# slinderman/pyglm

Measured on AMD Instinct MI355X. Metric: Gibbs sweeps/sec (full resample_model), higher is better.
Workload: dtype f64 (likelihood Gram: exact integer arithmetic on 13 i8 residue planes, CRT back to f64)

## Files before the change

### include/pyglm_hip.h

```cpp
#ifndef PYGLM_HIP_H
#define PYGLM_HIP_H
#include <stddef.h>
#include <stdint.h>
#ifdef __cplusplus
extern "C" {
#endif

#define PGL_ABI_VERSION 11

int pgl_abi_version(void);
const char* pgl_last_error(void);

int pgl_philox_words(uint64_t seed, uint32_t purpose, uint32_t j, uint64_t elem0, uint64_t stream, uint32_t* out, size_t n, void* hip_stream);

int pgl_pg_draw(const double* b, const double* z, double* out, size_t len, uint64_t seed, uint64_t stream, uint64_t elem0, void* hip_stream);

int pgl_design_matrix(const double* S, long lds, const double* basis, double* X, long ldx, double* Xt, long ldxt, int T, int N, int B, int R,
                      int clip, void* hip_stream);
int pgl_transpose(const double* src, long ld_src, double* dst, long ld_dst, int rows, int cols, void* hip_stream);

int pgl_activation(const double* Xt, long ldxt, const double* Wt, long ldw, double* Psi, long ldpsi, int T, int Dk, int nloc, void* hip_stream);

int pgl_pg_loglik(double* Psi, long ldpsi, const double* bias, const double* Y, long ldy, double* Omega, long ldo, double* Kappa, long ldk,
                  double* llpart, double* ll_out, int accumulate, int T, int nloc, int obs, double xi, uint64_t seed, uint64_t sweep,
                  uint64_t neuron0, uint64_t elem0, void* hip_stream);
int pgl_pg_loglik_partials(int T);
int pgl_pg_loglik_ex(double* Psi, long ldpsi, const double* bias, const double* Y, long ldy, double* Omega, long ldo, double* Kappa, long ldk,
                     double* llpart, double* ll_out, int accumulate, int T, int nloc, int obs, double xi, const double* param, const double* hooks,
                     long ldh, uint64_t seed, uint64_t sweep, uint64_t neuron0, uint64_t elem0, void* hip_stream);

int pgl_gaussian_stats(double* Psi, long ldpsi, const double* bias, const double* Y, long ldy, const double* inv_eta, double* Omega, long ldo,
                       double* Kappa, long ldk, double* part, double* sse_out, int accumulate, int T, int nloc, void* hip_stream);

int pgl_scaled_gram(const double* G0, long ldg, const double* inv_eta, double* J, long ldj, long strideJ, int D, int nz, void* hip_stream);

int pgl_weighted_gram(const double* X, long ldx, int x_cols, const double* W, long ldw, int Tp, int D, int nz, double* J, long ldj, long strideJ,
                      int accumulate, void* hip_stream);
int pgl_contract_tn(const double* A, long lda, int a_cols, const double* B, long ldb, int b_cols, double* C, long ldc, int M, int N, int K,
                    double alpha, double beta, void* hip_stream);
int pgl_contract_tn_batched(const double* A, long lda, long strideA, int a_cols, const double* B, long ldb, long strideB, int b_cols, double* C,
                            long ldc, long strideC, int M, int N, int K, int nbatch, const int* batch_k, double alpha, double beta, int tri,
                            int kernel, void* hip_stream);
int pgl_assemble_posterior(double* J, long ldj, long strideJ, const double* border_omega, const double* border_kappa, long ldb, const double* Jw,
                           const double* hw, const int* label, const double* Jb, const double* hb, int nb, int N, int B, void* hip_stream);

int pgl_i8_max_planes(void);
int pgl_i8_padded_rows(int D);
int pgl_i8_min_planes(int T);
int pgl_i8_norm_bits(int nplanes, int T);
double pgl_i8_norm_limit(int nplanes, int T);
size_t pgl_i8_plane_bytes(int D, int T);
size_t pgl_i8_residue_bytes(int D);
int pgl_i8_colstats(const double* X, long ldx, const double* Om, long ldo, int T, int D, int G, double* amax, double* sumsq, void* hip_stream);
int pgl_i8_scales(const double* amax, const double* sumsq, long ncols, int T, int nplanes, double* scale, void* hip_stream);
int pgl_i8_planes(const double* X, long ldx, const double* Om, long ldo, const double* scale, void* planes, int T, int D, int G, int nplanes,
                  long t0, void* hip_stream);
int pgl_i8_planes_t(const double* Xt, long ldt, const double* Om, long ldo, const double* scale, void* planes, int T, int D, int G, int nplanes,
                    long t0, void* hip_stream);
int pgl_i8_gram(const void* planes_x, const void* planes_wx, void* residues, int T, int D, int G, int nplanes, void* hip_stream);
int pgl_i8_gram_slice(const void* planes_x, int T_x, int t0, const void* planes_wx, void* residues, int T_slice, int T_total, int D, int G,
                      int nplanes, int accumulate, void* hip_stream);
int pgl_i8_crt(const void* residues, const double* scale_x, const double* scale_wx, double* J, long ldj, long strideJ, int T, int D, int G,
               int nplanes, int accumulate, void* hip_stream);

typedef struct {
    double* M; long ldj; long strideM;
    int nb, N, B;
    const int* perm;
    const double* u;
    const double* rho;
    const double* c0;
    int* a;
    const int* skip;
    int* d_idx; double* d_sign; int* d_cnt;
    int* batch_k;
    double* G;
    double* Lws;
    double* Ut; double* Wt; long ldu;
    int* status;
    int visit_order;
    double* logodds;
} pgl_flip_t;
int pgl_flip_kmax(void);
int pgl_flip_window_blocks(int B);
int pgl_flip_apply(const pgl_flip_t* s, void* hip_stream);
int pgl_flip_apply_chunk(const pgl_flip_t* s, int max_pivots, void* hip_stream);
int pgl_flip_apply_window(const pgl_flip_t* s, int window, void* hip_stream);
int pgl_flip_visit_order(const pgl_flip_t* s, const double* J, long ldj_src, long strideJ, void* hip_stream);
int pgl_flip_decide(const pgl_flip_t* s, int window, void* hip_stream);

typedef struct {
    const double* J; long ldj; long strideJ;
    const int* a;
    int* act; long ldact; int* na;
    double* Ac; long ldc; long strideC;
    double* hc;
    double* Tinv;
    const double* z; long ldz;
    double* W; double* b;
    int nb, N, B;
    int* status;
} pgl_chol_t;
int pgl_active_index(const pgl_chol_t* s, void* hip_stream);
int pgl_sample_weights(const pgl_chol_t* s, int na_max, void* hip_stream);

typedef struct {
    int T, Tp;
    const double* X;
    const double* Xt;
    const double* Y;
    double* Psi;
    double* OK;
    double* llpart;
    uint64_t elem0;
    int int8;
    int planes;
// ... 94 lines not shown
```

### pyglm_amd/_lib.py

```python
import ctypes
import os

_HERE = os.path.dirname(os.path.abspath(__file__))
LIB_PATH = os.path.join(_HERE, "lib", "libpyglm_hip.so")

c_p, c_l, c_i, c_d, c_u64, c_u32, c_sz = (ctypes.c_void_p, ctypes.c_long, ctypes.c_int, ctypes.c_double,
                                          ctypes.c_uint64, ctypes.c_uint32, ctypes.c_size_t)


class FlipState(ctypes.Structure):
    _fields_ = [("M", c_p), ("ldj", c_l), ("strideM", c_l), ("nb", c_i), ("N", c_i), ("B", c_i),
                ("perm", c_p), ("u", c_p), ("rho", c_p), ("c0", c_p), ("a", c_p), ("skip", c_p),
                ("d_idx", c_p), ("d_sign", c_p), ("d_cnt", c_p), ("batch_k", c_p), ("G", c_p), ("Lws", c_p),
                ("Ut", c_p), ("Wt", c_p), ("ldu", c_l), ("status", c_p), ("visit_order", c_i), ("logodds", c_p)]


class CholState(ctypes.Structure):
    _fields_ = [("J", c_p), ("ldj", c_l), ("strideJ", c_l), ("a", c_p), ("act", c_p), ("ldact", c_l), ("na", c_p),
                ("Ac", c_p), ("ldc", c_l), ("strideC", c_l), ("hc", c_p), ("Tinv", c_p), ("z", c_p), ("ldz", c_l),
                ("W", c_p), ("b", c_p), ("nb", c_i), ("N", c_i), ("B", c_i), ("status", c_p)]


class Dataset(ctypes.Structure):
    _fields_ = [("T", c_i), ("Tp", c_i), ("X", c_p), ("Xt", c_p), ("Y", c_p), ("Psi", c_p), ("OK", c_p), ("llpart", c_p), ("elem0", c_u64),
                ("int8", c_i), ("planes", c_i), ("sA", c_p), ("PA", c_p), ("omega_override", c_p), ("xmax", c_p),
                ("hooks", c_p)]


NSTAGES = 16


class StageTimes(ctypes.Structure):
    _fields_ = [("ms", c_d * NSTAGES), ("work", c_d * NSTAGES), ("calls", c_i * NSTAGES), ("pending", c_p), ("mask", c_u32)]


class Sweep(ctypes.Structure):
    _fields_ = [("N", c_i), ("B", c_i), ("n0", c_i), ("nloc", c_i), ("nb", c_i), ("obs", c_i), ("xi", c_d), ("visit_order", c_i),
                ("planes", c_i), ("i8_group", c_i), ("datasets", ctypes.POINTER(Dataset)), ("ndatasets", c_i),
                ("a", c_p), ("W", c_p), ("b", c_p), ("rho", c_p), ("Jw", c_p), ("hw", c_p), ("label", c_p), ("Jb", c_p), ("hb", c_p), ("c0", c_p),
                ("perm", c_p), ("u", c_p), ("z", c_p), ("inv_eta", c_p), ("G0", c_p), ("ll", c_p), ("status", c_p), ("logodds", c_p),
                ("Wt", c_p), ("bias", c_p), ("border", c_p), ("skip", c_p), ("c0_dense", c_p),
                ("Jbuf", c_p), ("Mtab", c_p), ("Ac", c_p), ("hc", c_p), ("Tinv", c_p), ("G", c_p), ("Lws", c_p), ("Ut", c_p), ("Wt_ws", c_p),
                ("d_idx", c_p), ("d_sign", c_p), ("d_cnt", c_p), ("batch_k", c_p), ("act", c_p), ("na", c_p),
                ("i8_PB", c_p), ("i8_R", c_p), ("i8_stat", c_p), ("i8_slice", c_i), ("i8_PAs", c_p), ("i8_Rx", c_p), ("i8_norm", c_p), ("nrun", c_i), ("nfirst", c_i),
                ("all_deterministic", c_i), ("init_rows_bound", c_i), ("active_rows_bound", c_i), ("flip_single_pass", c_i),
                ("times", ctypes.POINTER(StageTimes)), ("obs_param", c_p)]


SIGNATURES = {
    "pgl_abi_version": [],
    "pgl_last_error": [],
    "pgl_philox_words": [c_u64, c_u32, c_u32, c_u64, c_u64, c_p, c_sz, c_p],
    "pgl_pg_draw": [c_p, c_p, c_p, c_sz, c_u64, c_u64, c_u64, c_p],
    "pgl_design_matrix": [c_p, c_l, c_p, c_p, c_l, c_p, c_l, c_i, c_i, c_i, c_i, c_i, c_p],
    "pgl_transpose": [c_p, c_l, c_p, c_l, c_i, c_i, c_p],
    "pgl_activation": [c_p, c_l, c_p, c_l, c_p, c_l, c_i, c_i, c_i, c_p],
    "pgl_pg_loglik": [c_p, c_l, c_p, c_p, c_l, c_p, c_l, c_p, c_l, c_p, c_p, c_i, c_i, c_i, c_i, c_d, c_u64, c_u64, c_u64, c_u64, c_p],
    "pgl_pg_loglik_partials": [c_i],
    "pgl_pg_loglik_ex": [c_p, c_l, c_p, c_p, c_l, c_p, c_l, c_p, c_l, c_p, c_p, c_i, c_i, c_i, c_i, c_d, c_p, c_p, c_l, c_u64, c_u64, c_u64, c_u64, c_p],
    "pgl_gaussian_stats": [c_p, c_l, c_p, c_p, c_l, c_p, c_p, c_l, c_p, c_l, c_p, c_p, c_i, c_i, c_i, c_p],
    "pgl_scaled_gram": [c_p, c_l, c_p, c_p, c_l, c_l, c_i, c_i, c_p],
    "pgl_weighted_gram": [c_p, c_l, c_i, c_p, c_l, c_i, c_i, c_i, c_p, c_l, c_l, c_i, c_p],
    "pgl_i8_plane_bytes": [c_i, c_i],
    "pgl_i8_residue_bytes": [c_i],
    "pgl_i8_max_planes": [],
    "pgl_i8_padded_rows": [c_i],
    "pgl_i8_min_planes": [c_i],
    "pgl_i8_norm_bits": [c_i, c_i],
    "pgl_i8_norm_limit": [c_i, c_i],
    "pgl_i8_colstats": [c_p, c_l, c_p, c_l, c_i, c_i, c_i, c_p, c_p, c_p],
    "pgl_i8_scales": [c_p, c_p, c_l, c_i, c_i, c_p, c_p],
    "pgl_i8_planes": [c_p, c_l, c_p, c_l, c_p, c_p, c_i, c_i, c_i, c_i, c_l, c_p],
    "pgl_i8_planes_t": [c_p, c_l, c_p, c_l, c_p, c_p, c_i, c_i, c_i, c_i, c_l, c_p],
    "pgl_i8_gram": [c_p, c_p, c_p, c_i, c_i, c_i, c_i, c_p],
    "pgl_i8_gram_slice": [c_p, c_i, c_i, c_p, c_p, c_i, c_i, c_i, c_i, c_i, c_i, c_p],
    "pgl_i8_crt": [c_p, c_p, c_p, c_p, c_l, c_l, c_i, c_i, c_i, c_i, c_i, c_p],
    "pgl_contract_tn": [c_p, c_l, c_i, c_p, c_l, c_i, c_p, c_l, c_i, c_i, c_i, c_d, c_d, c_p],
    "pgl_contract_tn_batched": [c_p, c_l, c_l, c_i, c_p, c_l, c_l, c_i, c_p, c_l, c_l, c_i, c_i, c_i, c_i, c_p, c_d, c_d, c_i, c_i, c_p],
    "pgl_assemble_posterior": [c_p, c_l, c_l, c_p, c_p, c_l, c_p, c_p, c_p, c_p, c_p, c_i, c_i, c_i, c_p],
    "pgl_flip_kmax": [],
    "pgl_flip_window_blocks": [c_i],
    "pgl_flip_apply": [ctypes.POINTER(FlipState), c_p],
    "pgl_flip_apply_chunk": [ctypes.POINTER(FlipState), c_i, c_p],
    "pgl_flip_apply_window": [ctypes.POINTER(FlipState), c_i, c_p],
    "pgl_flip_visit_order": [ctypes.POINTER(FlipState), c_p, c_l, c_l, c_p],
    "pgl_flip_decide": [ctypes.POINTER(FlipState), c_i, c_p],
    "pgl_row_stats": [c_p, c_p, c_p, c_i, c_i, c_i, c_i, c_p],
    "pgl_sweep_dims": [c_i, c_i, c_i, ctypes.POINTER(c_i), ctypes.POINTER(c_i), ctypes.POINTER(c_i)],
    "pgl_sweep": [ctypes.POINTER(Sweep), c_u64, c_u64, c_p],
    "pgl_sweep_gram": [ctypes.POINTER(Sweep), c_i, c_i, c_p],
    "pgl_get_state": [ctypes.POINTER(Sweep), c_p, c_p, c_p, c_p, c_p, c_p],
    "pgl_stage_name": [c_i],
    "pgl_stage_times_collect": [ctypes.POINTER(StageTimes)],
    "pgl_active_index": [ctypes.POINTER(CholState), c_p],
    "pgl_sample_weights": [ctypes.POINTER(CholState), c_i, c_p],
    "pgl_ubench_mfma": [c_i, c_d, ctypes.POINTER(c_d), ctypes.POINTER(c_d), c_p],
    "pgl_generate_work_bytes": [c_i, c_i],
    "pgl_summary_fold": [c_p, c_l, c_p, c_p, c_p, c_p, c_i, c_i, c_i, c_i, c_d, c_p, c_p, c_l, c_p, c_p, c_p, c_p, c_i, c_p, c_d, c_p, c_p, c_p, c_p, c_i, c_p],
    "pgl_summary_state": [c_p, c_p, c_l, c_p, c_p, c_p, c_p, c_p, c_p, c_i, c_i, c_i, c_i, c_p],
    "pgl_summary_colsum": [c_p, c_l, c_i, c_i, c_p, c_p, c_i, c_p],
    "pgl_generate": [c_p, c_p, c_p, c_i, c_i, c_i, c_i, c_d, c_p, c_p, c_p, c_l, c_i, c_p, c_p, c_p],
    "pgl_simulate_work_bytes": [c_i, c_i, c_i],
    "pgl_simulate": [c_p, c_p, c_p, c_i, c_i, c_i, c_p, c_p, c_i, c_l, c_u64, c_p, c_p, c_l, c_p, c_p, c_l, c_i, c_p, c_p, c_p],
    "pgl_lagged_work_bytes": [c_i, c_i, c_i, c_i],
    "pgl_lagged_products": [c_p, c_l, c_l, c_i, c_i, c_i, c_i, c_i, c_p, c_l, c_i, c_i, c_p, c_p, c_p],
}

ABI_VERSION = 11
_lib = None


class PglError(RuntimeError):
    pass


def load():
    global _lib
    if _lib is not None:
        return _lib
    if not os.path.exists(LIB_PATH):
        raise PglError("libpyglm_hip.so not found at %s -- build it with `python -c 'import __graft_entry__ as g; g.build()'` "
                       "or `make -C pyglm_amd/csrc` (there is no CPU fallback)" % LIB_PATH)
    import torch
    lib = ctypes.CDLL(LIB_PATH)
    for name, args in SIGNATURES.items():
        fn = getattr(lib, name)
        fn.argtypes = args
        fn.restype = (ctypes.c_char_p if name in ("pgl_last_error", "pgl_stage_name") else ctypes.c_size_t if name in ("pgl_i8_plane_bytes", "pgl_i8_residue_bytes", "pgl_generate_work_bytes", "pgl_simulate_work_bytes", "pgl_lagged_work_bytes")
                      else ctypes.c_double if name == "pgl_i8_norm_limit" else ctypes.c_int)
# ... 30 lines not shown
```

### pyglm_amd/csrc/pgl_api.hip

```cpp
#include "pgl_common.h"
#include "pgl_obs.h"
#include <cstdarg>
#include <cstdio>

static thread_local char g_err[512] = "";
void pgl_set_error(const char* fmt, ...) {
    va_list ap;
    va_start(ap, fmt);
    vsnprintf(g_err, sizeof(g_err), fmt, ap);
    va_end(ap);
}

int pgl_device() {
    int dev = 0;
    if (hipGetDevice(&dev) != hipSuccess || dev < 0) dev = 0;
    return dev;
}
int pgl_device_cus(int dev) {
    static std::atomic<int> cus[PGL_MAX_DEVICES];
    const int slot = dev & (PGL_MAX_DEVICES - 1);
    int n = cus[slot].load(std::memory_order_relaxed);
    if (n <= 0) {
        if (hipDeviceGetAttribute(&n, hipDeviceAttributeMultiprocessorCount, dev) != hipSuccess || n <= 0) n = 256;
        cus[slot].store(n, std::memory_order_relaxed);
// ... 153 lines not shown
    return pgl_k_assemble_post(J, ldj, strideJ, border_omega, border_kappa, ldb, Jw, hw, label, Jb, hb, nb, N, B, ST(st));
}

size_t pgl_i8_plane_bytes(int D, int T) { return pgl_k_i8_plane_bytes(D, T); }
size_t pgl_i8_residue_bytes(int D) { return pgl_k_i8_residue_bytes(D); }
int pgl_i8_max_planes(void) { return pgl_k_i8_max_planes(); }
int pgl_i8_padded_rows(int D) { return pgl_k_i8_padded_rows(D); }
int pgl_i8_min_planes(int T) { return pgl_k_i8_min_planes(T); }
int pgl_i8_norm_bits(int nplanes, int T) { return pgl_k_i8_nu(nplanes, T); }
double pgl_i8_norm_limit(int nplanes, int T) { return pgl_k_i8_norm_limit(nplanes, T); }
#define PGL_CHECK_PLANES(np, T) PGL_CHECK_ARG((np) >= 1 && (np) <= pgl_k_i8_max_planes() && pgl_k_i8_nu((np), (T)) >= 8)
int pgl_i8_colstats(const double* X, long ldx, const double* Om, long ldo, int T, int D, int G, double* amax, double* sumsq, void* st) {
    PGL_CHECK_ARG(X && amax && sumsq && T > 0 && D > 0 && G >= 1 && G <= 8 && ldx >= D && (Om == nullptr ? G == 1 : ldo >= G));
    return pgl_k_i8_colstats(X, ldx, Om, ldo, T, D, G, amax, sumsq, ST(st));
}
int pgl_i8_scales(const double* amax, const double* sumsq, long ncols, int T, int nplanes, double* scale, void* st) {
    PGL_CHECK_ARG(amax && sumsq && scale && ncols > 0 && T > 0);
    PGL_CHECK_PLANES(nplanes, T);
    return pgl_k_i8_scales(amax, sumsq, ncols, T, nplanes, scale, ST(st));
}
int pgl_i8_planes(const double* X, long ldx, const double* Om, long ldo, const double* scale, void* planes, int T, int D, int G, int nplanes,
                  long t0, void* st) {
    PGL_CHECK_ARG(X && scale && planes && T > 0 && D > 0 && G > 0 && ldx >= D && (Om == nullptr || ldo >= G) && t0 >= 0);
    PGL_CHECK_ARG(Om != nullptr || G == 1);
    PGL_CHECK_PLANES(nplanes, T);
    return pgl_k_i8_planes(X, ldx, 0, Om, ldo, scale, static_cast<int8_t*>(planes), T, D, G, nplanes, t0, ST(st));
}
int pgl_i8_planes_t(const double* Xt, long ldt, const double* Om, long ldo, const double* scale, void* planes, int T, int D, int G, int nplanes,
                    long t0, void* st) {
    PGL_CHECK_ARG(Xt && scale && planes && T > 0 && D > 0 && G > 0 && ldt >= T && (Om == nullptr || ldo >= G) && t0 >= 0);
    PGL_CHECK_ARG(Om != nullptr || G == 1);
    PGL_CHECK_PLANES(nplanes, T);
    return pgl_k_i8_planes(Xt, ldt, 1, Om, ldo, scale, static_cast<int8_t*>(planes), T, D, G, nplanes, t0, ST(st));
}
int pgl_i8_gram(const void* planes_x, const void* planes_wx, void* residues, int T, int D, int G, int nplanes, void* st) {
    PGL_CHECK_ARG(planes_x && planes_wx && residues && T > 0 && D > 0 && G > 0);
    PGL_CHECK_PLANES(nplanes, T);
    return pgl_k_i8_gram(static_cast<const int8_t*>(planes_x), 0, 0, static_cast<const int8_t*>(planes_wx), static_cast<int8_t*>(residues), nullptr, T, D, G,
                         nplanes, 0, ST(st));
}
int pgl_i8_gram_slice(const void* planes_x, int T_x, int t0, const void* planes_wx, void* residues, int T_slice, int T_total, int D, int G, int nplanes,
                      int accumulate, void* st) {
    PGL_CHECK_ARG(planes_x && planes_wx && residues && T_slice > 0 && D > 0 && G > 0 && t0 >= 0 && t0 % 64 == 0 && T_total >= T_slice);
    PGL_CHECK_ARG(T_x == 0 || t0 + T_slice <= T_x);
    PGL_CHECK_PLANES(nplanes, T_total);
    return pgl_k_i8_gram(static_cast<const int8_t*>(planes_x), T_x > 0 ? pgl_k_i8_kp(T_x) : 0, T_x > 0 ? t0 / 64 : 0, static_cast<const int8_t*>(planes_wx),
                         static_cast<int8_t*>(residues), nullptr, T_slice, D, G, nplanes, accumulate, ST(st));
}
int pgl_i8_crt(const void* residues, const double* scale_x, const double* scale_wx, double* J, long ldj, long strideJ, int T, int D, int G,
               int nplanes, int accumulate, void* st) {
    PGL_CHECK_ARG(residues && scale_x && scale_wx && J && T > 0 && D > 0 && G > 0 && ldj >= D);
    PGL_CHECK_PLANES(nplanes, T);
    return pgl_k_i8_crt(static_cast<const int8_t*>(residues), nullptr, scale_x, scale_wx, J, ldj, strideJ, D, G, nplanes, accumulate, ST(st));
}

int pgl_summary_fold(const double* Psi, long ldn, const double* bias, const double* Y, double* llpart, double* ll_out, int accumulate, int T,
                     int nloc, int obs, double xi, const double* param, const double* hooks, long ldh, const double* inv_eta, double* rate_mean,
                     double* rate_M2, const int* link, int link0, const double* link_par, double link_par0, double* l_mean, double* l_M2,
                     double* lse_m, double* lse_s, int k, void* st) {
    PGL_CHECK_ARG(Psi && Y && llpart && ll_out && T > 0 && nloc > 0 && ldn >= nloc && obs >= 0 && obs <= 4 && k >= 1);
    PGL_CHECK_ARG(obs != 2 || inv_eta != nullptr);
    PGL_CHECK_ARG(obs == 2 || param != nullptr || obs == 0 || obs == 4 || (obs == 1 ? xi > 0 : xi >= 0));
    PGL_CHECK_ARG(obs != 4 || (hooks != nullptr && ldh >= nloc));
    PGL_CHECK_ARG((rate_mean == nullptr) == (rate_M2 == nullptr) && (link != nullptr || (link0 >= 0 && link0 <= 3)));
    PGL_CHECK_ARG((l_mean != nullptr) == (l_M2 != nullptr) && (l_mean != nullptr) == (lse_m != nullptr) && (l_mean != nullptr) == (lse_s != nullptr));
    PglSummaryFold f{};
    f.Psi = const_cast<double*>(Psi); f.ldpsi = ldn; f.bias = bias; f.Y = Y; f.ldy = ldn; f.llpart = llpart; f.T = T; f.nloc = nloc;
    f.obs = obs; f.xi = xi; f.param = param; f.hooks = obs == 4 ? hooks : nullptr; f.ldh = ldh; f.inv_eta = inv_eta;
    f.ll_out = ll_out; f.accumulate = accumulate;
    f.rmean = rate_mean; f.rM2 = rate_M2; f.link = link; f.link0 = link0; f.link_par = link_par; f.link_par0 = link_par0;
    f.lmean = l_mean; f.lM2 = l_M2; f.lse_m = lse_m; f.lse_s = lse_s; f.k = k;
    return pgl_k_summary_fold(f, ST(st));
}
int pgl_summary_state(const int* a, const double* Wt, long ldw, const double* bias, double* edge, double* w_mean, double* w_M2, double* b_mean,
                      double* b_M2, int N, int B, int nloc, int k, void* st) {
    PGL_CHECK_ARG(a && Wt && bias && edge && w_mean && w_M2 && b_mean && b_M2 && N > 0 && B > 0 && nloc > 0 && ldw >= nloc && k >= 1);
    return pgl_k_summary_state(a, Wt, ldw, bias, edge, w_mean, w_M2, b_mean, b_M2, N, B, nloc, k, ST(st));
}
int pgl_summary_colsum(const double* V, long ldv, int T, int nloc, double* part, double* out, int accumulate, void* st) {
    PGL_CHECK_ARG(V && part && out && T > 0 && nloc > 0 && ldv >= nloc);
    return pgl_k_summary_colsum(V, ldv, T, nloc, part, out, accumulate, ST(st));
}

int pgl_flip_kmax(void) { return pgl_k_flip_kmax(); }
int pgl_flip_window_blocks(int B) { return pgl_k_flip_window_blocks(B); }
int pgl_flip_apply(const pgl_flip_t* s, void* st) {
    PGL_CHECK_ARG(s && s->M && s->d_idx && s->d_sign && s->d_cnt && s->batch_k && s->G && s->Ut && s->Wt && s->status);
    PGL_CHECK_ARG(s->ldu >= (long)s->N * s->B + 2 && s->ldu % 2 == 0 && s->ldj >= (long)s->N * s->B + 2 && s->nb > 0);
    return pgl_k_flip_apply(*s, 0, 128, -1, ST(st));
}
int pgl_flip_apply_chunk(const pgl_flip_t* s, int max_pivots, void* st) {
    PGL_CHECK_ARG(s && s->M && s->d_idx && s->d_sign && s->d_cnt && s->batch_k && s->G && s->Lws && s->Ut && s->Wt && s->status);
    PGL_CHECK_ARG(s->ldu >= (long)s->N * s->B + 2 && s->ldu % 2 == 0 && s->ldj >= (long)s->N * s->B + 2 && s->nb > 0 && max_pivots > 0);
    return pgl_k_flip_apply(*s, 0, max_pivots, -1, ST(st));
}
int pgl_flip_visit_order(const pgl_flip_t* s, const double* J, long ldj_src, long strideJ, void* st) {
    PGL_CHECK_ARG(s && s->M && s->perm && J && s->visit_order && s->nb > 0 && ldj_src >= (long)s->N * s->B + 2 && s->ldj >= (long)s->N * s->B + 2);
    PGL_CHECK_ARG(s->B >= 1 && s->B <= 32);
    return pgl_k_flip_permute(*s, J, ldj_src, strideJ, ST(st));
}
int pgl_flip_apply_window(const pgl_flip_t* s, int window, void* st) {
    PGL_CHECK_ARG(s && s->M && s->d_idx && s->d_sign && s->d_cnt && s->batch_k && s->G && s->Ut && s->Wt && s->status);
    PGL_CHECK_ARG(s->ldu >= (long)s->N * s->B + 2 && s->ldu % 2 == 0 && s->ldj >= (long)s->N * s->B + 2 && s->nb > 0);
    PGL_CHECK_ARG(window >= 0);
    return pgl_k_flip_apply(*s, 1, 0, window, ST(st));
}
// ... 18 lines not shown
```

### pyglm_amd/csrc/pgl_common.h

```cpp
#pragma once
#include <hip/hip_runtime.h>
#include <stdint.h>
#include <stddef.h>
#include <atomic>
#include "../../include/pyglm_hip.h"

#define PGL_OK 0
#define PGL_ERR_ARG 1
#define PGL_ERR_HIP 2

void pgl_set_error(const char* fmt, ...);

#ifdef PGL_AB
#include <cstdlib>
inline int pgl_ab_int(const char* name, int dflt) { const char* e = getenv(name); return e ? atoi(e) : dflt; }
#else
constexpr int pgl_ab_int(const char*, int dflt) { return dflt; }
#endif

constexpr int PGL_MAX_DEVICES = 32;
int pgl_device();
int pgl_device_cus(int dev);
struct PglPerDevice {
    std::atomic<uint32_t> mask{0};
// ... 30 lines not shown
    double* C; long ldc; long strideC;
    const double* W; long ldw;
    int M, N, K;
    int a_cols, b_cols;
    int nbatch;
    int nz_total;
    double alpha, beta;
    int tri;
    const int* batch_k;
    int* sched;
    const int* batch_dim; int dim_off;
    int dim_mode;
    const int* batch_row_off;
    int pipe;
    int ksplit; long ks_rows; double* Cpart; long part_stride_z, part_stride_s;
};
enum PglGemmKind { PGL_GEMM_GRAM2 = 0, PGL_GEMM_PLAIN = 1, PGL_GEMM_TRI1 = 2, PGL_GEMM_SQUARES = 3 };
int pgl_launch_gemm(PglGemmKind kind, const PglGemmArgs& a, hipStream_t st);
int pgl_gram_split(const double* X, long ldx, int x_cols, const double* W, long ldw, int Tp, int D, int nz, double* J, long ldj, long strideJ, int accumulate,
                   long ks_rows, double* part, long part_stride_z, hipStream_t st);
bool pgl_update_supported(const PglGemmArgs& a);
int pgl_launch_update(const PglGemmArgs& a, hipStream_t st);
int pgl_launch_update_rows(const PglGemmArgs& a, int row0, int nrows, hipStream_t st);
int* pgl_sched_slot(hipStream_t st);

int pgl_k_philox_words(uint64_t, uint32_t, uint32_t, uint64_t, uint64_t, uint32_t*, size_t, hipStream_t);
int pgl_k_pg_draw(const double*, const double*, double*, size_t, uint64_t, uint64_t, uint64_t, hipStream_t);
int pgl_k_row_stats(const int* a, const double* W, double* out, int N, int B, int nloc, int n0, hipStream_t st);
int pgl_k_colsum_partials(const double* part, int nblk, int ncol, double* out, int accumulate, hipStream_t st);
int pgl_k_summary_state(const int* a, const double* Wt, long ldw, const double* bias, double* edge, double* wmean, double* wM2, double* bmean,
                        double* bM2, int N, int B, int nloc, int k, hipStream_t st);
int pgl_k_summary_colsum(const double* V, long ldv, int T, int nloc, double* part, double* out, int accumulate, hipStream_t st);
int pgl_k_scaled_gram(const double*, long, const double*, double*, long, long, int, int, hipStream_t);
int pgl_k_basis_conv(const double*, long, const double*, double*, long, double*, long, int, int, int, int, int, hipStream_t);
int pgl_k_transpose(const double*, long, double*, long, int, int, hipStream_t);
int pgl_k_assemble_post(double*, long, long, const double*, const double*, long, const double*, const double*, const int*, const double*,
                        const double*, int, int, int, hipStream_t);
size_t pgl_k_i8_plane_bytes(int, int);
size_t pgl_k_i8_residue_bytes(int);
int pgl_k_i8_max_planes(void);
int pgl_k_i8_padded_rows(int);
int pgl_k_i8_min_planes(int);
int pgl_k_i8_nu(int, int);
double pgl_k_i8_norm_limit(int, int);
int pgl_k_i8_colstats(const double*, long, const double*, long, int, int, int, double*, double*, hipStream_t);
int pgl_k_i8_scales(const double*, const double*, long, int, int, double*, hipStream_t);
int pgl_k_i8_colmax(const double*, long, int, int, double*, hipStream_t);
int pgl_k_i8_scales_bound(const double*, long, const double*, const double*, int, int, int, int, double*, hipStream_t);
int pgl_k_i8_colstats_scales(const double*, long, const double*, long, int, int, int, int, double*, double*, hipStream_t);
int pgl_k_i8_planes(const double*, long, int transposed, const double*, long, const double*, int8_t*, int, int, int, int, long t_base, hipStream_t);
int pgl_k_i8_gram(const int8_t*, long, int, const int8_t*, int8_t*, int8_t*, int, int, int, int, int, hipStream_t);
long pgl_k_i8_kp(int);
int pgl_k_i8_crt(const int8_t*, const int8_t*, const double*, const double*, double*, long, long, int, int, int, int, hipStream_t);
int pgl_k_flip_apply(const pgl_flip_t&, int, int, int, hipStream_t);
int pgl_k_flip_apply_pair(const pgl_flip_t&, int phase, int window, int* ws, hipStream_t);
int pgl_k_flip_permute(const pgl_flip_t&, const double*, long, long, hipStream_t);
int pgl_k_flip_decide(const pgl_flip_t&, int, hipStream_t);
int pgl_k_flip_pivot_list(const pgl_flip_t&, int*, long, int*, hipStream_t);
int pgl_k_flip_pivot_chunk(const pgl_flip_t&, const int*, long, const int*, int, int, hipStream_t);
int pgl_k_flip_kmax(void);
int pgl_k_flip_window_blocks(int);
int pgl_k_chol_index(const pgl_chol_t&, hipStream_t);
bool pgl_k_small_fits(int N, int B);
int pgl_k_small_max_rows(void);
int pgl_k_small_tail(const double* J, long ldj, long strideJ, int nb, int N, int B, const int* perm, const double* u, const double* rho, const double* c0,
                     int* a, const int* skip, const double* z, long ldz, double* W, double* b, int* status, double* logodds, hipStream_t st);
int pgl_k_chol_sample(const pgl_chol_t&, int, hipStream_t);
```

### pyglm_amd/csrc/pgl_i8gram.hip

```cpp
#include "pgl_common.h"
#include <cmath>
#include <type_traits>

namespace {

constexpr int NP = 15;
struct ModTable {
    int p[NP] = {256, 255, 253, 251, 247, 241, 239, 233, 229, 227, 223, 217, 211, 199, 197};
    int w[NP][NP] = {};
    int pinv[NP] = {};
    constexpr ModTable() {
        for (int q = 1; q < NP; ++q) {
            int prod = 1;
            for (int k = 0; k < q; ++k) {
                w[k][q] = prod > p[q] / 2 ? prod - p[q] : prod;
                prod = (prod * (p[k] % p[q])) % p[q];
            }
            int x = 1;
            while ((prod * x) % p[q] != 1) ++x;
            pinv[q] = x;
        }
    }
};
constexpr ModTable MT{};
__constant__ int c_mod[NP] = {256, 255, 253, 251, 247, 241, 239, 233, 229, 227, 223, 217, 211, 199, 197};

typedef int v4i __attribute__((ext_vector_type(4)));
typedef int v16i __attribute__((ext_vector_type(16)));
typedef __attribute__((address_space(3))) void* lds_ptr_t;
typedef const __attribute__((address_space(1))) void* glb_ptr_t;

constexpr int ELEM_BITS = 50;

constexpr int CS_COLS = 16, CS_LANES = 64, CS_G = 8, CS_ROWS = 4;
template <int G, bool WEIGHTED>
__global__ __launch_bounds__(CS_COLS * CS_LANES) void i8_colstats_kernel(const double* __restrict__ X, long ldx, const double* __restrict__ Om,
                                                                        long ldo, int T, int D, double* __restrict__ amax,
                                                                        double* __restrict__ ss) {
    constexpr int CH = CS_LANES * CS_ROWS;
    __shared__ double red[2][CS_LANES][CS_COLS + 1];
    __shared__ double oms[WEIGHTED ? CH : 1][WEIGHTED ? G : 1];
    const int tid = threadIdx.x, cl = tid % CS_COLS, tl = tid / CS_COLS, c = blockIdx.x * CS_COLS + cl;
    const bool live = c < D;
    const int tchunk = ((T + (int)gridDim.y - 1) / (int)gridDim.y + CH - 1) / CH * CH;
    const int tbeg = (int)blockIdx.y * tchunk;
    T = T < tbeg + tchunk ? T : tbeg + tchunk;
    amax += (long)blockIdx.y * G * D;
    ss += (long)blockIdx.y * G * D;
    double m[G], q[G];
#pragma unroll
    for (int g = 0; g < G; ++g) { m[g] = 0.0; q[g] = 0.0; }
    for (int t0 = tbeg; t0 < T; t0 += CH) {
        if (WEIGHTED) {
            __syncthreads();
            for (int e = tid; e < CH * G; e += CS_COLS * CS_LANES) {
                const int t = t0 + e / G;
                oms[e / G][e % G] = t < T ? Om[(long)t * ldo + e % G] : 0.0;
            }
            __syncthreads();
        }
        double x[CS_ROWS];
#pragma unroll
        for (int r = 0; r < CS_ROWS; ++r) {
            const int t = t0 + tl + r * CS_LANES;
            x[r] = (live && t < T) ? X[(long)t * ldx + c] : 0.0;
        }
#pragma unroll
        for (int r = 0; r < CS_ROWS; ++r)
#pragma unroll
            for (int g = 0; g < G; ++g) {
                const double v = WEIGHTED ? x[r] * oms[tl + r * CS_LANES][g] : x[r];
                m[g] = fmax(m[g], fabs(v));
                q[g] = fma(v, v, q[g]);
// ... 467 lines not shown
    asm volatile("s_getreg_b32 %0, hwreg(HW_REG_XCC_ID)" : "=s"(xcc));
    xcc &= 7u;
    for (;;) {
        __syncthreads();
        if (threadIdx.x == 0) {
            int w = -1, y = 0;
            for (int hop = 0; hop < 8 && w < 0; ++hop) {
                y = (int)((xcc + hop) & 7u);
                const int it = atomicAdd(&g.sched[y], 1);
                if (npx) { if (it < per_xcd) w = it; }
                else {
                    const long cand = ((long)(it / CH) * 8 + y) * CH + it % CH;
                    if (cand < total) w = (int)cand;
                }
            }
            if (w >= 0) {
                int tm, tn, gz, q, kpart = -1, tile;
                if (!npx) { const int pair = w / ntiles; tile = w % ntiles; gz = pair / g.np; q = pair % g.np; }
                else if (pieces) {
                    const int per_piece = npx * ntiles, per_plane = PGL_KPARTS(g) * per_piece, r = w % per_plane, r2 = r % per_piece;
                    q = w / per_plane; kpart = r / per_piece; gz = y + 8 * (r2 / ntiles); tile = r2 % ntiles;
                }
                else if (w < nfull) {
                    const int per_plane = npx * ntiles, r = w % per_plane;
                    q = w / per_plane; gz = y + 8 * (r / ntiles); tile = r % ntiles;
                } else {
                    const int r0 = w - nfull, j = r0 / (4 * ntiles), r = r0 % (4 * ntiles), grp = r / 128, within = r - grp * 128;
                    const int tg = min(32, ntiles - grp * 32);
                    kpart = within / tg;
                    tile = grp * 32 + within % tg;
                    gz = y + 8 * j; q = g.np - 1;
                }
                clustered_tile(tile, ntm, g.sbr, g.sbc, tm, tn);
                ticket[1] = gz; ticket[2] = tm; ticket[3] = tn; ticket[4] = kpart; ticket[5] = q;
            }
            ticket[0] = w;
        }
        __syncthreads();
        if (ticket[0] < 0) break;
        const int gz = __builtin_amdgcn_readfirstlane(ticket[1]), q = __builtin_amdgcn_readfirstlane(ticket[5]);
        const int tm = __builtin_amdgcn_readfirstlane(ticket[2]), tn = __builtin_amdgcn_readfirstlane(ticket[3]);
        const int kpart = __builtin_amdgcn_readfirstlane(ticket[4]);
        __syncthreads();
        i8_gram_item_big(g, gz, q, tm, tn, lds, kpart);
    }
}

struct CrtArgs {
    const int8_t* R;
    const double* sA; const double* sB;
    double* J; long ldj; long strideJ;
    int D, Dq, G, accumulate, np;
    const int8_t* Rx;
};

__device__ __forceinline__ double recip_scale(double x) {
    const long long b = __double_as_longlong(x);
    const bool pow2 = (b & 0x000FFFFFFFFFFFFFll) == 0 && b > 0x0010000000000000ll && b < 0x7FD0000000000000ll;
    return pow2 ? __longlong_as_double(0x7FE0000000000000ll - b) : 1.0 / x;
}

__global__ __launch_bounds__(256) void i8_crt_kernel(CrtArgs a) {
    const int j0 = (blockIdx.x * 256 + threadIdx.x) * 4, i = blockIdx.y, gz = blockIdx.z;
    if (j0 > i || i >= a.D) return;
    const int8_t* R = a.R + ((long)gz * a.np) * a.Dq * a.Dq + (long)i * a.Dq + j0;
    int w[NP];
#pragma unroll
    for (int q = 0; q < NP; ++q) w[q] = q < a.np ? *reinterpret_cast<const int*>(R + (long)q * a.Dq * a.Dq) : 0;
    int wx[3] = {0, 0, 0};
    if (a.Rx) {
        const int8_t* Rx = a.Rx + (long)gz * 3 * a.Dq * a.Dq + (long)i * a.Dq + j0;
#pragma unroll
        for (int k = 0; k < 3; ++k) wx[k] = *reinterpret_cast<const int*>(Rx + (long)k * a.Dq * a.Dq);
    }
    const double ra = recip_scale(a.sA[i]);
    double out[4];
#pragma unroll
    for (int e = 0; e < 4; ++e) {
        int v[NP];
#pragma unroll
        for (int q = 0; q < NP; ++q) v[q] = (int)(int8_t)((unsigned)w[q] >> (8 * e));
        if (a.Rx) {
            const int x = (int)(int8_t)((unsigned)wx[0] >> (8 * e)) + (int)(int8_t)((unsigned)wx[1] >> (8 * e)) + (int)(int8_t)((unsigned)wx[2] >> (8 * e));
#pragma unroll
            for (int q = 1; q < NP; ++q) if (q == a.np - 1) v[q] += x;
        }
#pragma unroll
        for (int q = 1; q < NP; ++q) {
            if (q < a.np) {
                const int p = MT.p[q];
                int u = v[q];
#pragma unroll
                for (int k = 0; k < q; ++k) u -= v[k] * MT.w[k][q];
                int t = u * MT.pinv[q] % p;
                if (t > p / 2) t -= p; else if (t < -(p / 2)) t += p;
                v[q] = t;
            }
        }
        double s = 0.0;
#pragma unroll
        for (int q = NP - 1; q >= 0; --q)
            if (q < a.np) s = s * (double)MT.p[q] + (double)v[q];
        const int j = j0 + e;
        const double rb = j < a.D ? recip_scale(a.sB[(long)gz * a.D + j]) : 0.0;
        out[e] = (s * ra) * rb;
    }
    double* dst = a.J + (long)gz * a.strideJ + (long)i * a.ldj + j0;
    if (j0 + 3 <= i && !a.accumulate && (reinterpret_cast<uintptr_t>(dst) % 16 == 0)) {
        *reinterpret_cast<d2_t*>(dst) = d2_t{out[0], out[1]};
        *reinterpret_cast<d2_t*>(dst + 2) = d2_t{out[2], out[3]};
    } else {
#pragma unroll
        for (int e = 0; e < 4; ++e)
            if (j0 + e <= i) dst[e] = a.accumulate ? dst[e] + out[e] : out[e];
    }
}

}

int pgl_k_i8_padded_rows(int D) { return (D + BT - 1) / BT * BT; }

static long pgl_i8_kp(int T) { const long k = ((long)T + 63) / 64 * 64; return k < 256 ? 256 : k; }

double pgl_k_i8_norm_limit(int nplanes, int T) {
    double l2 = 0.0;
    for (int q = 0; q < nplanes && q < NP; ++q) l2 += std::log2((double)MT.p[q]);
    const double lim = (std::exp2((l2 - 1.0) * 0.5) - std::sqrt((double)(T < 1 ? 1 : T)) - 1.0) / (1.0 + 1e-9);
    return lim > 0.0 ? lim : 0.0;
}
int pgl_k_i8_nu(int nplanes, int T) {
    const double lim = pgl_k_i8_norm_limit(nplanes, T);
    if (!(lim >= 2.0)) return 0;
    return (int)std::floor(std::log2(lim) - 1e-12);
}
int pgl_k_i8_max_planes(void) { return NP; }
int pgl_k_i8_min_planes(int T) {
    for (int k = 1; k <= NP; ++k)
        if (pgl_k_i8_nu(k, T) >= 50) return k;
    return NP + 1;
}

long pgl_k_i8_kp(int T) { return pgl_i8_kp(T); }
static int pgl_k_i8_kparts() { static const int v = pgl_ab_int("PGL_I8_KPARTS", 0); return v >= 2 && v <= 16 ? v : 0; }
static bool pgl_k_i8_split(int G, int nplanes) { return G % 8 == 0 && nplanes >= 2 && pgl_k_i8_kparts() == 0; }
size_t pgl_k_i8_plane_bytes(int D, int T) {
    const long Dq = pgl_k_i8_padded_rows(D), Kp = pgl_i8_kp(T);
    return (size_t)NP * Dq * Kp;
}
size_t pgl_k_i8_residue_bytes(int D) {
    const long Dq = pgl_k_i8_padded_rows(D);
    return (size_t)NP * Dq * Dq;
}

int pgl_k_i8_colstats(const double* X, long ldx, const double* Om, long ldo, int T, int D, int G, double* amax, double* ss, hipStream_t st) {
    if (G > CS_G || G < 1) { pgl_set_error("i8 colstats: %d weight columns per call (max %d)", G, CS_G); return PGL_ERR_ARG; }
    const dim3 grid((D + CS_COLS - 1) / CS_COLS), block(CS_COLS * CS_LANES);
#define PGL_CS(g_) case g_: hipLaunchKernelGGL((i8_colstats_kernel<g_, true>), grid, block, 0, st, X, ldx, Om, ldo, T, D, amax, ss); break;
    if (!Om) hipLaunchKernelGGL((i8_colstats_kernel<1, false>), grid, block, 0, st, X, ldx, Om, ldo, T, D, amax, ss);
    else switch (G) { PGL_CS(1) PGL_CS(2) PGL_CS(3) PGL_CS(4) PGL_CS(5) PGL_CS(6) PGL_CS(7) PGL_CS(8) default: break; }
#undef PGL_CS
    PGL_CHECK_LAUNCH();
    return PGL_OK;
}

constexpr int CS_NCH = 4;
int pgl_k_i8_colstats_scales(const double* X, long ldx, const double* Om, long ldo, int T, int D, int G, int nplanes, double* scratch, double* scale,
                             hipStream_t st) {
    if (G > CS_G || G < 1 || !Om) { pgl_set_error("i8 colstats+scales: %d weight columns per call (max %d)", G, CS_G); return PGL_ERR_ARG; }
// ... 34 lines not shown
    if (pgl_k_i8_nu(nplanes, T) < 8) { pgl_set_error("i8 scales: %d moduli leave no room for T = %d", nplanes, T); return PGL_ERR_ARG; }
    hipLaunchKernelGGL(i8_scales_kernel, dim3((unsigned)((n + 255) / 256)), dim3(256), 0, st, amax, ss, n, pgl_k_i8_norm_limit(nplanes, T), scale, 1);
    PGL_CHECK_LAUNCH();
    return PGL_OK;
}

int pgl_k_i8_planes(const double* X, long ldx, int transposed, const double* Om, long ldo, const double* scale, int8_t* P, int T, int D, int G,
                    int nplanes, long t_base, hipStream_t st) {
    const int Dq = pgl_k_i8_padded_rows(D);
    const long Kp = pgl_i8_kp(T);
    const bool aligned = (ldx % 2 == 0) && (reinterpret_cast<uintptr_t>(X) % 16 == 0);
    for (int g0 = 0; g0 < G; g0 += CS_G) {
        const int gz = G - g0 < CS_G ? G - g0 : CS_G;
        PlaneArgs a{X, ldx, transposed, Om ? Om + g0 : nullptr, ldo, scale + (long)g0 * D, P + (long)g0 * nplanes * Dq * Kp, T, D, Dq, Kp, nplanes, (unsigned)t_base};
        if (transposed && aligned)
            hipLaunchKernelGGL(i8_planes_t_kernel<256>, dim3((unsigned)((Kp + 255) / 256), Dq / PT_D), dim3(256), 0, st, a, gz);
        else
            hipLaunchKernelGGL(i8_planes_kernel<512>, dim3((unsigned)((Kp + 511) / 512), Dq / PT_D), dim3(512), 0, st, a, gz);
        PGL_CHECK_LAUNCH();
    }
    return PGL_OK;
}

int pgl_k_i8_gram(const int8_t* PA, long KpA, int ka0, const int8_t* PB, int8_t* R, int8_t* Rx, int T, int D, int G, int nplanes, int accumulate, hipStream_t st) {
    const int Dq = pgl_k_i8_padded_rows(D);
    const long Kp = pgl_i8_kp(T);
    if (KpA <= 0) { KpA = Kp; ka0 = 0; }
    const int nkt = (T + BKB - 1) / BKB;
    if (KpA % BKB != 0 || (long)(ka0 + nkt) * BKB > KpA) { pgl_set_error("i8 gram: slice of %d tiles at tile %d outside the X planes (%ld bytes per row)", nkt, ka0, KpA); return PGL_ERR_ARG; }
    static PglPerDevice attr;
    if (int rc = pgl_set_dynamic_lds(reinterpret_cast<const void*>(i8_gram_kernel), BNST * BSTAGE, attr)) return rc;
    const int n_cu = pgl_device_cus(pgl_device());
    const int ntm = Dq / BT, ntiles = ntm * (ntm + 1) / 2;
    const long total = (long)ntiles * nplanes * G;
    if (total <= 0) return PGL_OK;
    if (total * 4 > 0x7fffffffL) { pgl_set_error("i8 gram: %ld work items", total); return PGL_ERR_ARG; }
    const unsigned grid = (unsigned)(total < n_cu ? total : n_cu);
    const bool lists = G % 8 == 0;
    static const int sbr_ab = pgl_ab_int("PGL_I8_SBR", 0), sbc_ab = pgl_ab_int("PGL_I8_SBC", 0);
    const int sbr = sbr_ab > 0 ? sbr_ab : (lists ? ntm : SB), sbc = sbc_ab > 0 ? sbc_ab : (lists ? 2 : SB);
    for (int kt0 = 0; kt0 < nkt; kt0 += KCH) {
        GramArgs g{PA, PB, R, Dq, Kp, G, nplanes, sbr, sbc, nkt, kt0, pgl_sched_slot(st), KpA, ka0, accumulate ? 1 : 0, pgl_k_i8_split(G, nplanes) ? Rx : nullptr, lists ? pgl_k_i8_kparts() : 0};
        if (!g.sched) { pgl_set_error("i8 gram: scheduler scratch unavailable"); return PGL_ERR_HIP; }
        hipLaunchKernelGGL(i8_gram_kernel, dim3(grid), dim3(256), BNST * BSTAGE, st, g);
        PGL_CHECK_LAUNCH();
    }
    return PGL_OK;
}

int pgl_k_i8_crt(const int8_t* R, const int8_t* Rx, const double* sA, const double* sB, double* J, long ldj, long strideJ, int D, int G, int nplanes,
                 int accumulate, hipStream_t st) {
    const int Dq = pgl_k_i8_padded_rows(D);
    if (G <= 0) return PGL_OK;
    CrtArgs c{R, sA, sB, J, ldj, strideJ, D, Dq, G, accumulate, nplanes, (Rx != nullptr && pgl_k_i8_split(G, nplanes)) ? Rx : nullptr};
    hipLaunchKernelGGL(i8_crt_kernel, dim3((D + 1023) / 1024, D, G), dim3(256), 0, st, c);
    PGL_CHECK_LAUNCH();
    return PGL_OK;
}
```

Measured before the change: 0.05904.

## Rewrite i8 CRT reconstruction with float vectorized residues and triangular tile grid

The CRT kernel now does the mixed-radix digit reduction in vectorized float4 arithmetic, using precomputed pinv-folded weights and rintf rounding, instead of integer multiply and modulo per element. The launch grid covers only lower-triangular BT tiles split into 16-row slabs, instead of a D x ceil(D/1024) grid with mostly idle threads. The kernel is templated on the plane count so the loops fully unroll. It also adds a split-residue API, a standalone reduce kernel for testing, and an A/B probe mode. The float reduction relies on the intermediates staying exactly representable in float.

Measured after the change: 0.05944 (median of 6 runs). About the same (+0.7%).

```diff
diff --git a/include/pyglm_hip.h b/include/pyglm_hip.h
--- a/include/pyglm_hip.h
+++ b/include/pyglm_hip.h
@@ -62,6 +62,9 @@
                       int nplanes, int accumulate, void* hip_stream);
 int pgl_i8_crt(const void* residues, const double* scale_x, const double* scale_wx, double* J, long ldj, long strideJ, int T, int D, int G,
                int nplanes, int accumulate, void* hip_stream);
+int pgl_i8_crt_split(const void* residues, const void* residues_x, const double* scale_x, const double* scale_wx, double* J, long ldj,
+                     long strideJ, int T, int D, int G, int nplanes, int accumulate, void* hip_stream);
+int pgl_i8_crt_reduce(const int* u, int* digit, long n, int q, void* hip_stream);
 
 typedef struct {
     double* M; long ldj; long strideM;
diff --git a/pyglm_amd/_lib.py b/pyglm_amd/_lib.py
--- a/pyglm_amd/_lib.py
+++ b/pyglm_amd/_lib.py
@@ -75,6 +75,8 @@
     "pgl_i8_gram": [c_p, c_p, c_p, c_i, c_i, c_i, c_i, c_p],
     "pgl_i8_gram_slice": [c_p, c_i, c_i, c_p, c_p, c_i, c_i, c_i, c_i, c_i, c_i, c_p],
     "pgl_i8_crt": [c_p, c_p, c_p, c_p, c_l, c_l, c_i, c_i, c_i, c_i, c_i, c_p],
+    "pgl_i8_crt_split": [c_p, c_p, c_p, c_p, c_p, c_l, c_l, c_i, c_i, c_i, c_i, c_i, c_p],
+    "pgl_i8_crt_reduce": [c_p, c_p, c_l, c_i, c_p],
     "pgl_contract_tn": [c_p, c_l, c_i, c_p, c_l, c_i, c_p, c_l, c_i, c_i, c_i, c_d, c_d, c_p],
     "pgl_contract_tn_batched": [c_p, c_l, c_l, c_i, c_p, c_l, c_l, c_i, c_p, c_l, c_l, c_i, c_i, c_i, c_i, c_p, c_d, c_d, c_i, c_i, c_p],
     "pgl_assemble_posterior": [c_p, c_l, c_l, c_p, c_p, c_l, c_p, c_p, c_p, c_p, c_p, c_i, c_i, c_i, c_p],
diff --git a/pyglm_amd/csrc/pgl_api.hip b/pyglm_amd/csrc/pgl_api.hip
--- a/pyglm_amd/csrc/pgl_api.hip
+++ b/pyglm_amd/csrc/pgl_api.hip
@@ -229,6 +229,17 @@
     PGL_CHECK_ARG(residues && scale_x && scale_wx && J && T > 0 && D > 0 && G > 0 && ldj >= D);
     PGL_CHECK_PLANES(nplanes, T);
     return pgl_k_i8_crt(static_cast<const int8_t*>(residues), nullptr, scale_x, scale_wx, J, ldj, strideJ, D, G, nplanes, accumulate, ST(st));
+}
+int pgl_i8_crt_split(const void* residues, const void* residues_x, const double* scale_x, const double* scale_wx, double* J, long ldj, long strideJ,
+                     int T, int D, int G, int nplanes, int accumulate, void* st) {
+    PGL_CHECK_ARG(residues && residues_x && scale_x && scale_wx && J && T > 0 && D > 0 && G > 0 && ldj >= D);
+    PGL_CHECK_PLANES(nplanes, T);
+    return pgl_k_i8_crt(static_cast<const int8_t*>(residues), static_cast<const int8_t*>(residues_x), scale_x, scale_wx, J, ldj, strideJ, D, G, nplanes,
+                        accumulate, ST(st));
+}
+int pgl_i8_crt_reduce(const int* u, int* digit, long n, int q, void* st) {
+    PGL_CHECK_ARG(u && digit && n > 0 && q >= 1 && q < pgl_k_i8_max_planes());
+    return pgl_k_i8_crt_reduce(u, digit, n, q, ST(st));
 }
 
 int pgl_summary_fold(const double* Psi, long ldn, const double* bias, const double* Y, double* llpart, double* ll_out, int accumulate, int T,
diff --git a/pyglm_amd/csrc/pgl_common.h b/pyglm_amd/csrc/pgl_common.h
--- a/pyglm_amd/csrc/pgl_common.h
+++ b/pyglm_amd/csrc/pgl_common.h
@@ -106,6 +106,7 @@
 int pgl_k_i8_gram(const int8_t*, long, int, const int8_t*, int8_t*, int8_t*, int, int, int, int, int, hipStream_t);
 long pgl_k_i8_kp(int);
 int pgl_k_i8_crt(const int8_t*, const int8_t*, const double*, const double*, double*, long, long, int, int, int, int, hipStream_t);
+int pgl_k_i8_crt_reduce(const int*, int*, long, int, hipStream_t);
 int pgl_k_flip_apply(const pgl_flip_t&, int, int, int, hipStream_t);
 int pgl_k_flip_apply_pair(const pgl_flip_t&, int phase, int window, int* ws, hipStream_t);
 int pgl_k_flip_permute(const pgl_flip_t&, const double*, long, long, hipStream_t);
diff --git a/pyglm_amd/csrc/pgl_i8gram.hip b/pyglm_amd/csrc/pgl_i8gram.hip
--- a/pyglm_amd/csrc/pgl_i8gram.hip
+++ b/pyglm_amd/csrc/pgl_i8gram.hip
@@ -9,6 +9,9 @@
     int p[NP] = {256, 255, 253, 251, 247, 241, 239, 233, 229, 227, 223, 217, 211, 199, 197};
     int w[NP][NP] = {};
     int pinv[NP] = {};
+    int wf[NP][NP] = {};
+    int pf[NP] = {};
+    static constexpr int sym(int x, int m) { x %= m; return x > m / 2 ? x - m : x < -(m / 2) ? x + m : x; }
     constexpr ModTable() {
         for (int q = 1; q < NP; ++q) {
             int prod = 1;
@@ -19,6 +22,8 @@
             int x = 1;
             while ((prod * x) % p[q] != 1) ++x;
             pinv[q] = x;
+            pf[q] = sym(x, p[q]);
+            for (int k = 0; k < q; ++k) wf[k][q] = sym(w[k][q] * x, p[q]);
         }
     }
 };
@@ -592,6 +597,12 @@
     double* J; long ldj; long strideJ;
     int D, Dq, G, accumulate, np;
     const int8_t* Rx;
+#ifdef PGL_AB
+#define PGL_CRT_PROBE(a_) ((a_).probe)
+#else
+#define PGL_CRT_PROBE(a_) 0
+#endif
+    int probe;
 };
 
 __device__ __forceinline__ double recip_scale(double x) {
@@ -600,60 +611,108 @@
     return pow2 ? __longlong_as_double(0x7FE0000000000000ll - b) : 1.0 / x;
 }
 
+typedef float f4_t __attribute__((ext_vector_type(4)));
+
+template <typename F>
+__device__ __forceinline__ F crt_reduce(F u, int Q) {
+    const float p = (float)MT.p[Q], ip = 1.0f / (float)MT.p[Q];
+    F q = u * ip;
+    if constexpr (std::is_same<F, float>::value) q = rintf(q);
+    else {
+#pragma unroll
+        for (int e = 0; e < 4; ++e) q[e] = rintf(q[e]);
+    }
+    return u - p * q;
+}
+__device__ __forceinline__ double crt_horner(double s, double p, double v) {
+#pragma clang fp contract(off)
+    const double m = s * p;
+    return m + v;
+}
+__device__ __forceinline__ f4_t crt_bytes(int w) {
+    return f4_t{(float)(int8_t)w, (float)(int8_t)((unsigned)w >> 8), (float)(int8_t)((unsigned)w >> 16), (float)(w >> 24)};
+}
+
+constexpr int CRT_ROWS = 16, CRT_SLABS = BT / CRT_ROWS;
+template <int NPT>
 __global__ __launch_bounds__(256) void i8_crt_kernel(CrtArgs a) {
-    const int j0 = (blockIdx.x * 256 + threadIdx.x) * 4, i = blockIdx.y, gz = blockIdx.z;
-    if (j0 > i || i >= a.D) return;
-    const int8_t* R = a.R + ((long)gz * a.np) * a.Dq * a.Dq + (long)i * a.Dq + j0;
-    int w[NP];
-#pragma unroll
-    for (int q = 0; q < NP; ++q) w[q] = q < a.np ? *reinterpret_cast<const int*>(R + (long)q * a.Dq * a.Dq) : 0;
-    int wx[3] = {0, 0, 0};
-    if (a.Rx) {
-        const int8_t* Rx = a.Rx + (long)gz * 3 * a.Dq * a.Dq + (long)i * a.Dq + j0;
-#pragma unroll
-        for (int k = 0; k < 3; ++k) wx[k] = *reinterpret_cast<const int*>(Rx + (long)k * a.Dq * a.Dq);
-    }
-    const double ra = recip_scale(a.sA[i]);
-    double out[4];
-#pragma unroll
-    for (int e = 0; e < 4; ++e) {
-        int v[NP];
-#pragma unroll
-        for (int q = 0; q < NP; ++q) v[q] = (int)(int8_t)((unsigned)w[q] >> (8 * e));
+    const int np = NPT ? NPT : a.np;
+    const int gz = blockIdx.y, slab = blockIdx.x % CRT_SLABS, tile = blockIdx.x / CRT_SLABS;
+    const int tm = isqrt_tri_i(tile), tn = tile - tm * (tm + 1) / 2;
+    const int i0 = tm * BT + slab * CRT_ROWS;
+    if (i0 >= a.D) return;
+    const int W = tm == tn ? (CRT_ROWS / 4) * (slab + 1) : BT / 4;
+    const float rW = 1.0f / (float)W;
+    const long plane = (long)a.Dq * a.Dq;
+    for (int e0 = threadIdx.x; e0 < CRT_ROWS * W; e0 += 256) {
+        const int rr = (int)(((float)e0 + 0.5f) * rW);
+        const int i = i0 + rr, j0 = tn * BT + 4 * (e0 - rr * W);
+        if (i >= a.D || j0 > i) continue;
+        const int8_t* R = a.R + ((long)gz * np) * plane + (long)i * a.Dq + j0;
+        int w[NP];
+#pragma unroll
+        for (int q = 0; q < NP; ++q) {
+            if (PGL_CRT_PROBE(a) == 2) w[q] = q < np ? (int)((unsigned)(j0 + 7 * q + i) * 0x01010101u) : 0;
+            else w[q] = q < np ? *reinterpret_cast<const int*>(R + (long)q * plane) : 0;
+        }
+        int wx[3] = {0, 0, 0};
+        if (a.Rx && PGL_CRT_PROBE(a) != 2) {
+            const int8_t* Rx = a.Rx + (long)gz * 3 * plane + (long)i * a.Dq + j0;
+#pragma unroll
+            for (int k = 0; k < 3; ++k) wx[k] = *reinterpret_cast<const int*>(Rx + (long)k * plane);
+        }
+        f4_t v[NP];
+#pragma unroll
+        for (int q = 0; q < NP; ++q) v[q] = crt_bytes(w[q]);
         if (a.Rx) {
-            const int x = (int)(int8_t)((unsigned)wx[0] >> (8 * e)) + (int)(int8_t)((unsigned)wx[1] >> (8 * e)) + (int)(int8_t)((unsigned)wx[2] >> (8 * e));
-#pragma unroll
-            for (int q = 1; q < NP; ++q) if (q == a.np - 1) v[q] += x;
-        }
-#pragma unroll
-        for (int q = 1; q < NP; ++q) {
-            if (q < a.np) {
-                const int p = MT.p[q];
-                int u = v[q];
-#pragma unroll
-                for (int k = 0; k < q; ++k) u -= v[k] * MT.w[k][q];
-                int t = u * MT.pinv[q] % p;
-                if (t > p / 2) t -= p; else if (t < -(p / 2)) t += p;
-                v[q] = t;
-            }
-        }
-        double s = 0.0;
-#pragma unroll
-        for (int q = NP - 1; q >= 0; --q)
-            if (q < a.np) s = s * (double)MT.p[q] + (double)v[q];
-        const int j = j0 + e;
-        const double rb = j < a.D ? recip_scale(a.sB[(long)gz * a.D + j]) : 0.0;
-        out[e] = (s * ra) * rb;
-    }
-    double* dst = a.J + (long)gz * a.strideJ + (long)i * a.ldj + j0;
-    if (j0 + 3 <= i && !a.accumulate && (reinterpret_cast<uintptr_t>(dst) % 16 == 0)) {
-        *reinterpret_cast<d2_t*>(dst) = d2_t{out[0], out[1]};
-        *reinterpret_cast<d2_t*>(dst + 2) = d2_t{out[2], out[3]};
-    } else {
-#pragma unroll
-        for (int e = 0; e < 4; ++e)
-            if (j0 + e <= i) dst[e] = a.accumulate ? dst[e] + out[e] : out[e];
-    }
+            const f4_t x = crt_bytes(wx[0]) + crt_bytes(wx[1]) + crt_bytes(wx[2]);
+#pragma unroll
+            for (int q = 1; q < NP; ++q) if (q == np - 1) v[q] += x;
+        }
+        if (PGL_CRT_PROBE(a) != 1) {
+#pragma unroll
+            for (int q = 1; q < NP; ++q) {
+                if (q < np) {
+                    f4_t u = v[q] * (float)MT.pf[q];
+#pragma unroll
+                    for (int k = 0; k < q; ++k) u -= v[k] * (float)MT.wf[k][q];
+                    v[q] = crt_reduce(u, q);
+                }
+            }
+        }
+        const double ra = recip_scale(a.sA[i]);
+        double out[4];
+#pragma unroll
+        for (int e = 0; e < 4; ++e) {
+            double s = 0.0;
+#pragma unroll
+            for (int q = NP - 1; q >= 0; --q)
+                if (q < np) s = crt_horner(s, (double)MT.p[q], (double)v[q][e]);
+            const int j = j0 + e;
+            const double rb = j < a.D ? recip_scale(a.sB[(long)gz * a.D + j]) : 0.0;
+            out[e] = (s * ra) * rb;
+        }
+        double* dst = a.J + (long)gz * a.strideJ + (long)i * a.ldj + j0;
+        if (j0 + 3 <= i && !a.accumulate && (reinterpret_cast<uintptr_t>(dst) % 16 == 0)) {
+            *reinterpret_cast<d2_t*>(dst) = d2_t{out[0], out[1]};
+            *reinterpret_cast<d2_t*>(dst + 2) = d2_t{out[2], out[3]};
+        } else {
+#pragma unroll
+            for (int e = 0; e < 4; ++e)
+                if (j0 + e <= i) dst[e] = a.accumulate ? dst[e] + out[e] : out[e];
+        }
+    }
+}
+
+__global__ __launch_bounds__(256) void i8_crt_reduce_kernel(const int* __restrict__ u, int* __restrict__ digit, long n, int q) {
+    const long k = (long)blockIdx.x * 256 + threadIdx.x;
+    if (k >= n) return;
+    const float x = (float)u[k];
+    float t = 0.f;
+#pragma unroll
+    for (int qq = 1; qq < NP; ++qq)
+        if (qq == q) t = crt_reduce(x, qq);
+    digit[k] = (int)t;
 }
 
 }
@@ -794,8 +853,24 @@
                  int accumulate, hipStream_t st) {
     const int Dq = pgl_k_i8_padded_rows(D);
     if (G <= 0) return PGL_OK;
-    CrtArgs c{R, sA, sB, J, ldj, strideJ, D, Dq, G, accumulate, nplanes, (Rx != nullptr && pgl_k_i8_split(G, nplanes)) ? Rx : nullptr};
-    hipLaunchKernelGGL(i8_crt_kernel, dim3((D + 1023) / 1024, D, G), dim3(256), 0, st, c);
+    static const int probe = pgl_ab_int("PGL_CRT_PROBE", 0);
+    CrtArgs c{R, sA, sB, J, ldj, strideJ, D, Dq, G, accumulate, nplanes, (Rx != nullptr && pgl_k_i8_split(G, nplanes)) ? Rx : nullptr, probe};
+    const int ntm = (D + BT - 1) / BT;
+    const dim3 grid((unsigned)(ntm * (ntm + 1) / 2 * CRT_SLABS), (unsigned)G);
+    switch (nplanes) {
+        case 12: hipLaunchKernelGGL(i8_crt_kernel<12>, grid, dim3(256), 0, st, c); break;
+        case 13: hipLaunchKernelGGL(i8_crt_kernel<13>, grid, dim3(256), 0, st, c); break;
+        case 14: hipLaunchKernelGGL(i8_crt_kernel<14>, grid, dim3(256), 0, st, c); break;
+        case 15: hipLaunchKernelGGL(i8_crt_kernel<15>, grid, dim3(256), 0, st, c); break;
+        default: hipLaunchKernelGGL(i8_crt_kernel<0>, grid, dim3(256), 0, st, c); break;
+    }
     PGL_CHECK_LAUNCH();
     return PGL_OK;
 }
+
+int pgl_k_i8_crt_reduce(const int* u, int* digit, long n, int q, hipStream_t st) {
+    if (q < 1 || q >= NP) { pgl_set_error("i8 crt reduce: modulus index %d outside 1..%d", q, NP - 1); return PGL_ERR_ARG; }
+    hipLaunchKernelGGL(i8_crt_reduce_kernel, dim3((unsigned)((n + 255) / 256)), dim3(256), 0, st, u, digit, n, q);
+    PGL_CHECK_LAUNCH();
+    return PGL_OK;
+}
```
